# Jackxiini/Pytorch-distributed-learning

Measured on AMD Instinct MI355X. Metric: images/sec (whole node) MNIST ConvNet at 1/2/4/8 MI355X; DDP scaling efficiency, higher is better.
Workload: dtype bf16

## Files before the change

csrc/kernels/convnet.hip:

```cpp
#include <algorithm>
#include <cstdlib>
#include <type_traits>
#include <vector>

#include <cstdio>
#include <cstdlib>

#include "device_common.h"
#include "kernels.h"
#include "sgd_device.h"

namespace ringdp {
namespace kern {

using namespace ringdp::dev;

namespace {

__host__ __device__ constexpr int cdiv(int a, int b) { return (a + b - 1) / b; }

constexpr int P1_OFF = 0, P1_N = 2 * 2 * 512;
constexpr int P2F_OFF = P1_OFF + P1_N, P2F_N = 4 * 9 * 512;
constexpr int P3F_OFF = P2F_OFF + P2F_N, P3F_N = 8 * 18 * 512;
constexpr int P2D_OFF = P3F_OFF + P3F_N, P2D_N = 2 * 18 * 512;
// ... 2046 lines not shown
  __shared__ __attribute__((aligned(16))) uint8_t lds[C1W_LDS];
  bf16* xs = reinterpret_cast<bf16*>(lds + C1W_XS);
  const int tid = threadIdx.x, lane = tid & 63, wave = tid >> 6;
  const int i16 = lane & 15, g = lane >> 4, q = i16 >> 2, p = i16 & 3;
  const int t1 = 16 + i16;
  const int xoff0 = (i16 % 5) * C1W_CS + (i16 / 5) * C1W_RS + 8 * g;
  const int xoff1 = t1 < 25 ? (t1 % 5) * C1W_CS + (t1 / 5) * C1W_RS + 8 * g : 0;
  const uint32_t b1fill = t1 == 25 ? 0x3f803f80u : 0u;
  for (int i = tid; i < C1W_C / 16; i += 256) reinterpret_cast<uint4*>(lds)[i] = make_uint4(0, 0, 0, 0);
  const int per = cdiv(B, nslices);
  const int b_lo = min(B, blockIdx.x * per), b_hi = min(B, b_lo + per);
  auto dma = [&](int bb, int k) {
    const bf16* src = da1 + (int64_t)bb * C1A_IMG;
    uint8_t* dd = lds + C1W_D + k * C1W_DSZ;
    for (int i = wave; i < 11; i += 4) {
      const int c = i * 64 + lane;
      if (c < C1A_IMG / 8) glds16_async(src + c * 8, dd + i * 1024);
    }
    const uint8_t* cs = idx1 + (int64_t)bb * C1I_IMG;
    uint8_t* cd = lds + C1W_C + k * C1I_IMG;
    for (int i = wave; i < 7; i += 4) {
      const int c = i * 64 + lane;
      if (c < C1I_IMG / 16) glds16_async(cs + c * 16, cd + i * 1024);
    }
  };
  f32x4 acc[2][2];
#pragma unroll
  for (int m = 0; m < 2; ++m) acc[m][0] = acc[m][1] = zero_f32x4();
  uint32_t xu = 0;
  float4 xf = make_float4(0.f, 0.f, 0.f, 0.f);
  __syncthreads();
  if (b_lo < b_hi) {
    c1_load<U8>(xin, b_lo, tid, xu, xf);
    dma(b_lo, 0);
    c1_store<U8, 5, C1W_RS, C1W_CS>(xs, tid, xu, xf, mean, inv_std, in_scale);
  }
  int cur = 0;
  for (int b = b_lo; b < b_hi; ++b) {
    c_dma_wait();
    __syncthreads();
    if (b + 1 < b_hi) {
      c1_load<U8>(xin, b + 1, tid, xu, xf);
      dma(b + 1, cur ^ 1);
    }
    const bf16* D = reinterpret_cast<const bf16*>(lds + C1W_D + cur * C1W_DSZ);
    const uint8_t* CB = lds + C1W_C + cur * C1I_IMG;
    const int dy = wave & 1;
    for (int ks = wave; ks < 26; ks += 4) {
      const int py = ks >> 1;
      bf16x8 A[2];
#pragma unroll
      for (int m = 0; m < 2; ++m) {
        const uint2 d = __builtin_bit_cast(uint2, lds_read_tr16(D + (py * 13 + 4 * g + q) * 32 + m * 16 + 4 * p));
        const int co = m * 16 + i16;
        const uint32_t cu = *reinterpret_cast<const uint32_t*>(CB + py * 256 + (co >> 1) * 16 + 4 * g);
        const int csh = 4 * (co & 1) + 2 * dy;
        uint32_t pr[4];
#pragma unroll
        for (int k = 0; k < 4; ++k) {
          const uint32_t dv = k & 1 ? (k < 2 ? d.x : d.y) >> 16 : (k < 2 ? d.x : d.y) & 0xffffu;
          const uint32_t sel = __builtin_amdgcn_ubfe(cu, 8 * k + csh, 2);
          pr[k] = dv * ((sel * 0x8001u) & 0x10001u);
        }
        A[m] = __builtin_bit_cast(bf16x8, make_uint4(pr[0], pr[1], pr[2], pr[3]));
      }
      const bf16x8 B0 = *reinterpret_cast<const bf16x8*>(xs + xoff0 + ks * C1W_RS);
      bf16x8 B1 = *reinterpret_cast<const bf16x8*>(xs + xoff1 + ks * C1W_RS);
      if (t1 >= 25) B1 = __builtin_bit_cast(bf16x8, make_uint4(b1fill, b1fill, b1fill, b1fill));
#pragma unroll
      for (int m = 0; m < 2; ++m) {
        acc[m][0] = mfma16x16x32(A[m], B0, acc[m][0]);
        acc[m][1] = mfma16x16x32(A[m], B1, acc[m][1]);
      }
    }
    if (b + 1 < b_hi) {
      __syncthreads();
      c1_store<U8, 5, C1W_RS, C1W_CS>(xs, tid, xu, xf, mean, inv_std, in_scale);
    }
    cur ^= 1;
  }
  __syncthreads();
  float* red = reinterpret_cast<float*>(lds);
#pragma unroll
  for (int m = 0; m < 2; ++m)
#pragma unroll
    for (int n = 0; n < 2; ++n)
      *reinterpret_cast<f32x4*>(red + ((wave * 4 + m * 2 + n) * 64 + lane) * 4) = acc[m][n];
  __syncthreads();
  const int tile = tid >> 6;
  f32x4 sum = *reinterpret_cast<const f32x4*>(red + (tile * 64 + lane) * 4);
#pragma unroll
  for (int w = 1; w < 4; ++w) sum += *reinterpret_cast<const f32x4*>(red + ((w * 4 + tile) * 64 + lane) * 4);
  float* slab = slabs + (int64_t)blockIdx.x * C1_WSLAB;
  const int tap = (tile & 1) * 16 + i16;
#pragma unroll
  for (int r = 0; r < 4; ++r) {
    const int co = (tile >> 1) * 16 + g * 4 + r;
    if (tap < 25) slab[co * 25 + tap] = sum[r];
    if (tap == 25) slab[800 + co] = sum[r];
  }
}

constexpr int C12_O = 172 * C2_ORS * 2;
constexpr int C12_XS = 5 * C1W_CS * 2;
constexpr int C12_OFF_O = C2D_P, C12_OFF_X = C12_OFF_O + 2 * C12_O, C12_OFF_C = C12_OFF_X + 2 * C12_XS;
constexpr int C12_LDS = C12_OFF_C + 2 * C1I_IMG;
constexpr int C12B_LDS = C12_LDS > (C2W_D + C2W_X) ? C12_LDS : (C2W_D + C2W_X);
static_assert(C2D_P % 16 == 0 && C12_O % 16 == 0 && C12_XS % 16 == 0, "16-B aligned LDS buffers");
static_assert(8 * 4 * 64 * 4 * 4 <= C12_OFF_X, "conv1 cross-wave reduction fits in P + O");

template <bool U8>
__device__ __forceinline__ void conv12_dgrad_role(char* smem, const void* __restrict__ xin, const uint8_t* __restrict__ idx1,
                                  const bf16* __restrict__ dz2, const bf16* __restrict__ packed, int B, int block,
                                  int nblocks, float mean, float inv_std, float in_scale,
                                  float* __restrict__ slabs1) {
  bf16* P = reinterpret_cast<bf16*>(smem);
  auto Obuf = [&](int k) { return reinterpret_cast<bf16*>(smem + C12_OFF_O + k * C12_O); };
  auto Xbuf = [&](int k) { return reinterpret_cast<bf16*>(smem + C12_OFF_X + k * C12_XS); };
  auto Cbuf = [&](int k) { return reinterpret_cast<uint8_t*>(smem + C12_OFF_C + k * C1I_IMG); };
  const int tid = threadIdx.x, lane = tid & 63, wave = tid >> 6;
  const int nt = wave & 1, mg = wave >> 1;
  const int r16 = lane & 15, q8 = (lane >> 4) * 8;
  const bf16x8* pk = reinterpret_cast<const bf16x8*>(packed + P2D_OFF);
  bf16x8 bw[18];
#pragma unroll
  for (int ks = 0; ks < 18; ++ks) bw[ks] = pk[(nt * 18 + ks) * 64 + lane];
  int base[3];
  int opos[3][4];
#pragma unroll
  for (int k = 0; k < 3; ++k) {
    const int mt = min(mg + 4 * k, 10);
    const int mm = c2d_tile_pos[mt * 16 + r16] == 255 ? 0 : c2d_tile_pos[mt * 16 + r16];
    base[k] = (mm / 13) * C2_PW + mm % 13;
#pragma unroll
    for (int i = 0; i < 4; ++i) opos[k][i] = c2d_tile_pos[mt * 16 + (lane >> 4) * 4 + i];
  }
  const int i16 = lane & 15, g = lane >> 4, q = i16 >> 2, p = i16 & 3;
  const int t1 = 16 + i16;
  const int xoff0 = (i16 % 5) * C1W_CS + (i16 / 5) * C1W_RS + 8 * g;
  const int xoff1 = t1 < 25 ? (t1 % 5) * C1W_CS + (t1 / 5) * C1W_RS + 8 * g : 0;
  const uint32_t b1fill = t1 == 25 ? 0x3f803f80u : 0u;
  const int dy = wave & 1;
  f32x4 acc1[2][2];
#pragma unroll
  for (int m = 0; m < 2; ++m) acc1[m][0] = acc1[m][1] = zero_f32x4();
  for (int c = tid; c < C12_OFF_C / 16; c += 512) reinterpret_cast<bf16x8*>(smem)[c] = zero_bf16x8();
  bf16x8 pz[2];
  uint4 pc = make_uint4(0, 0, 0, 0);
  uint32_t xu = 0;
  float4 xf = make_float4(0.f, 0.f, 0.f, 0.f);
  auto load = [&](int bb) {
    const bf16x8* src = reinterpret_cast<const bf16x8*>(dz2 + (int64_t)bb * 121 * 64);
    pz[0] = src[tid];
    if (tid + 512 < 968) pz[1] = src[tid + 512];
    if (tid < C1I_IMG / 16) pc = reinterpret_cast<const uint4*>(idx1 + (int64_t)bb * C1I_IMG)[tid];
    c1_load<U8>(xin, bb, tid, xu, xf);
  };
  auto stage = [&](int k) {
#pragma unroll
    for (int j = 0; j < 2; ++j) {
      const int c = tid + 512 * j;
      if (c < 968) {
        const int pos = c >> 3, cc = (c & 7) * 8;
        *reinterpret_cast<bf16x8*>(P + ((pos / 11 + 2) * C2_PW + pos % 11 + 2) * C2_PRS + cc) = pz[j];
      }
    }
    if (tid < C1I_IMG / 16) reinterpret_cast<uint4*>(Cbuf(k))[tid] = pc;
    c1_store<U8, 5, C1W_RS, C1W_CS>(Xbuf(k), tid, xu, xf, mean, inv_std, in_scale);
  };
  auto c1_step = [&](int j, int k) {
    const int ks0 = wave + 8 * j;
    const bool ok = ks0 < 26;
    const int ks = ok ? ks0 : 0;
    const int py = ks >> 1;
    const bf16* O = Obuf(k);
    const bf16* xs = Xbuf(k);
    const uint8_t* CB = Cbuf(k);
    bf16x8 A[2];
#pragma unroll
    for (int m = 0; m < 2; ++m) {
      const uint2 d = __builtin_bit_cast(uint2, lds_read_tr16(O + (py * 13 + 4 * g + q) * C2_ORS + m * 16 + 4 * p));
      const int co = m * 16 + i16;
      const uint32_t cu = *reinterpret_cast<const uint32_t*>(CB + py * 256 + (co >> 1) * 16 + 4 * g);
      const int csh = 4 * (co & 1) + 2 * dy;
      uint32_t pr[4];
#pragma unroll
      for (int e = 0; e < 4; ++e) {
        const uint32_t dv = e & 1 ? (e < 2 ? d.x : d.y) >> 16 : (e < 2 ? d.x : d.y) & 0xffffu;
        const uint32_t sel = __builtin_amdgcn_ubfe(cu, 8 * e + csh, 2);
        pr[e] = ok ? dv * ((sel * 0x8001u) & 0x10001u) : 0u;
      }
      A[m] = __builtin_bit_cast(bf16x8, make_uint4(pr[0], pr[1], pr[2], pr[3]));
    }
    const bf16x8 B0 = *reinterpret_cast<const bf16x8*>(xs + xoff0 + ks * C1W_RS);
    bf16x8 B1 = *reinterpret_cast<const bf16x8*>(xs + xoff1 + ks * C1W_RS);
    if (t1 >= 25) B1 = __builtin_bit_cast(bf16x8, make_uint4(b1fill, b1fill, b1fill, b1fill));
#pragma unroll
    for (int m = 0; m < 2; ++m) {
      acc1[m][0] = mfma16x16x32(A[m], B0, acc1[m][0]);
      acc1[m][1] = mfma16x16x32(A[m], B1, acc1[m][1]);
    }
  };
  auto phase = [&](auto nk_c, auto c1_c, int k) {
    constexpr int NK = decltype(nk_c)::value;
    constexpr bool C1 = decltype(c1_c)::value;
    f32x4 acc[NK];
#pragma unroll
    for (int m = 0; m < NK; ++m) acc[m] = zero_f32x4();
#pragma unroll
    for (int ks = 0; ks < 18; ++ks) {
      const int tapp = ks >> 1, c0 = (ks & 1) * 32;
      const int shift = (tapp / 3) * C2_PW + tapp % 3;
#pragma unroll
      for (int m = 0; m < NK; ++m)
        acc[m] = mfma16x16x32(*reinterpret_cast<const bf16x8*>(P + (base[m] + shift) * C2_PRS + c0 + q8), bw[ks],
                              acc[m]);
      if (C1 && (ks & 3) == 3 && ks < 16) c1_step(ks >> 2, k ^ 1);
    }
    bf16* O = Obuf(k);
#pragma unroll
    for (int m = 0; m < NK; ++m) {
#pragma unroll
      for (int i = 0; i < 4; ++i) {
        const int pos = opos[m][i];
        if (pos < 169) O[pos * C2_ORS + nt * 16 + r16] = (bf16)acc[m][i];
      }
    }
  };
  using I2 = std::integral_constant<int, 2>;
  using I3 = std::integral_constant<int, 3>;
  using T = std::true_type;
  using Fa = std::false_type;
  __syncthreads();
  int b = block, k = 0;
  if (b < B) load(b);
  for (int i = 0; b < B; ++i, b += nblocks, k ^= 1) {
    __syncthreads();
    stage(k);
    const int nb = b + nblocks;
    if (nb < B) load(nb);
    __syncthreads();
    if (i == 0) {
      if (mg < 3) phase(I3{}, Fa{}, k);
      else phase(I2{}, Fa{}, k);
    } else {
      if (mg < 3) phase(I3{}, T{}, k);
      else phase(I2{}, T{}, k);
    }
  }
  __syncthreads();
  if (b != block) {
#pragma unroll
    for (int j = 0; j < 4; ++j) c1_step(j, k ^ 1);
  }
  __syncthreads();
  float* red = reinterpret_cast<float*>(smem);
#pragma unroll
  for (int m = 0; m < 2; ++m)
#pragma unroll
    for (int n = 0; n < 2; ++n)
      *reinterpret_cast<f32x4*>(red + ((wave * 4 + m * 2 + n) * 64 + lane) * 4) = acc1[m][n];
  __syncthreads();
  if (tid >= 256) return;
  const int tile = tid >> 6;
  f32x4 sum = *reinterpret_cast<const f32x4*>(red + (tile * 64 + lane) * 4);
#pragma unroll
  for (int w = 1; w < 8; ++w) sum += *reinterpret_cast<const f32x4*>(red + ((w * 4 + tile) * 64 + lane) * 4);
  float* slab = slabs1 + (int64_t)block * C1_WSLAB;
  const int tap = (tile & 1) * 16 + i16;
#pragma unroll
  for (int r = 0; r < 4; ++r) {
    const int co = (tile >> 1) * 16 + g * 4 + r;
    if (tap < 25) slab[co * 25 + tap] = sum[r];
    if (tap == 25) slab[800 + co] = sum[r];
  }
}

template <bool U8>
__global__ __launch_bounds__(512) void conv12_bwd_kernel(const void* __restrict__ xin,
                                                         const uint8_t* __restrict__ idx1,
                                                         const bf16* __restrict__ a1,
                                                         const bf16* __restrict__ dz2,
                                                         const bf16* __restrict__ packed, int B,
                                                         float mean, float inv_std, float in_scale,
                                                         float* __restrict__ slabs2, int nslices,
                                                         float* __restrict__ slabs1, int n_dgrad) {
  __shared__ __attribute__((aligned(16))) char smem[C12B_LDS];
  if ((int)blockIdx.x < n_dgrad)
    conv12_dgrad_role<U8>(smem, xin, idx1, dz2, packed, B, blockIdx.x, n_dgrad, mean, inv_std, in_scale, slabs1);
  else
    conv2_wgrad_role(smem, a1, dz2, slabs2, B, nslices, blockIdx.x - n_dgrad);
}

constexpr int C12V_DG = 2 * (C2D_P + C12_O) + 3 * (C12_XS + C1I_IMG);
constexpr int C12V_WG = 3 * (C2W_D + C2W_X);
constexpr int C12V_LDS = C12V_DG > C12V_WG ? C12V_DG : C12V_WG;
static_assert(C12V_LDS <= 160 * 1024 && C1I_IMG % 16 == 0, "conv12 backward (8-wave) LDS");

#ifndef RINGDP_C12_ABLATE
#define RINGDP_C12_ABLATE 0
#endif
constexpr int C12_ABLATE = RINGDP_C12_ABLATE;

template <bool U8>
__device__ __forceinline__ void conv12_dgrad8_role(char* smem, const void* __restrict__ xin,
                                                   const uint8_t* __restrict__ idx1, const bf16* __restrict__ dz2,
                                                   const bf16* __restrict__ packed, int B, int block, int nblocks,
                                                   float mean, float inv_std, float in_scale,
                                                   float* __restrict__ slabs1, int ablate) {
  auto Pb = [&](int k) { return reinterpret_cast<bf16*>(smem + k * C2D_P); };
  auto Ob = [&](int k) { return reinterpret_cast<bf16*>(smem + 2 * C2D_P + k * C12_O); };
  auto Xb = [&](int k) { return reinterpret_cast<bf16*>(smem + 2 * (C2D_P + C12_O) + k * C12_XS); };
  auto Cb = [&](int k) { return reinterpret_cast<uint8_t*>(smem + 2 * (C2D_P + C12_O) + 3 * C12_XS + k * C1I_IMG); };
  const int tid = threadIdx.x, lane = tid & 63;
  const int wave = __builtin_amdgcn_readfirstlane(tid >> 6);
  const int n = block < B ? (B - block + nblocks - 1) / nblocks : 0;
  for (int c = tid; c < (2 * (C2D_P + C12_O) + 3 * C12_XS) / 16; c += 512)
    reinterpret_cast<bf16x8*>(smem)[c] = zero_bf16x8();
  __syncthreads();
  if ((ablate & 8) && wave >= 4) __builtin_amdgcn_s_setprio(1);
  if (wave < 4) {
    const int r16 = lane & 15, q8 = (lane >> 4) * 8, c4 = (lane >> 4) * 4;
    const bf16x8* pk = reinterpret_cast<const bf16x8*>(packed + P2D_OFF);
    bf16x8 bw[2][18];
#pragma unroll
    for (int nt = 0; nt < 2; ++nt)
#pragma unroll
      for (int ks = 0; ks < 18; ++ks) bw[nt][ks] = pk[(nt * 18 + ks) * 64 + lane];
    int base[3], opos[3];
#pragma unroll
    for (int k = 0; k < 3; ++k) {
      const int mt = min(wave + 4 * k, 10);
      const int mm = c2d_tile_pos[mt * 16 + r16];
      opos[k] = mm;
      base[k] = mm == 255 ? 0 : (mm / 13) * C2_PW + mm % 13;
    }
    auto phase = [&](auto nk_c, const bf16* P, bf16* O) {
      constexpr int NK = decltype(nk_c)::value;
      f32x4 acc[NK][2];
#pragma unroll
      for (int k = 0; k < NK; ++k) acc[k][0] = acc[k][1] = zero_f32x4();
#pragma unroll
      for (int ks = 0; ks < 18; ++ks) {
        const int tapp = ks >> 1, c0 = (ks & 1) * 32;
        const int shift = (tapp / 3) * C2_PW + tapp % 3;
#pragma unroll
        for (int k = 0; k < NK; ++k) {
          const bf16x8 a = *reinterpret_cast<const bf16x8*>(P + (base[k] + shift) * C2_PRS + c0 + q8);
          acc[k][0] = mfma16x16x32(bw[0][ks], a, acc[k][0]);
          acc[k][1] = mfma16x16x32(bw[1][ks], a, acc[k][1]);
        }
      }
#pragma unroll
      for (int k = 0; k < NK; ++k) {
        if (opos[k] < 169) {
#pragma unroll
          for (int nt = 0; nt < 2; ++nt)
            *reinterpret_cast<bf16x4*>(O + opos[k] * C2_ORS + nt * 16 + c4) =
                bf16x4{(bf16)acc[k][nt][0], (bf16)acc[k][nt][1], (bf16)acc[k][nt][2], (bf16)acc[k][nt][3]};
        }
      }
    };
    lds_barrier();
    for (int s = 0; s <= n; ++s) {
      if (s < n && !(ablate & 2)) {
        if (wave < 3)
          phase(std::integral_constant<int, 3>{}, Pb(s & 1), Ob(s & 1));
        else
          phase(std::integral_constant<int, 2>{}, Pb(s & 1), Ob(s & 1));
      }
      lds_barrier();
    }
    __syncthreads();
    __syncthreads();
  } else {
    const int vt = tid - 256, vw = wave - 4;
    const int i16 = lane & 15, g = lane >> 4, q = i16 >> 2, p = i16 & 3;
    const int t1 = 16 + i16;
    const int xoff0 = (i16 % 5) * C1W_CS + (i16 / 5) * C1W_RS + 8 * g;
    const int xoff1 = t1 < 25 ? (t1 % 5) * C1W_CS + (t1 / 5) * C1W_RS + 8 * g : 0;
    const uint32_t b1fill = t1 == 25 ? 0x3f803f80u : 0u;
    const int dy = vw & 1;
    f32x4 acc1[2][2];
#pragma unroll
    for (int m = 0; m < 2; ++m) acc1[m][0] = acc1[m][1] = zero_f32x4();
    struct Regs {
      bf16x8 pz[4];
      uint4 pc;
      uint32_t xu;
      float4 xf;
    };
    Regs r0, r1;
    auto load = [&](Regs& r, int bb) {
      const bf16x8* src = reinterpret_cast<const bf16x8*>(dz2 + (int64_t)bb * 121 * 64);
#pragma unroll
      for (int j = 0; j < 4; ++j)
        if (vt + 256 * j < 968) r.pz[j] = src[vt + 256 * j];
      if (vt < C1I_IMG / 16) r.pc = reinterpret_cast<const uint4*>(idx1 + (int64_t)bb * C1I_IMG)[vt];
      c1_load<U8>(xin, bb, vt, r.xu, r.xf);
    };
    auto stage = [&](const Regs& r, int k2, int k3) {
      bf16* P = Pb(k2);
#pragma unroll
      for (int j = 0; j < 4; ++j) {
        const int c = vt + 256 * j;
        if (c < 968) {
          const int pos = c >> 3, cc = (c & 7) * 8;
          *reinterpret_cast<bf16x8*>(P + ((pos / 11 + 2) * C2_PW + pos % 11 + 2) * C2_PRS + cc) = r.pz[j];
        }
      }
      if (vt < C1I_IMG / 16) reinterpret_cast<uint4*>(Cb(k3))[vt] = r.pc;
      c1_store<U8, 5, C1W_RS, C1W_CS>(Xb(k3), vt, r.xu, r.xf, mean, inv_std, in_scale);
    };
    auto c1_step = [&](int ks, const bf16* O, const bf16* xs, const uint8_t* CB) {
      const int py = ks >> 1;
      bf16x8 A[2];
#pragma unroll
      for (int m = 0; m < 2; ++m) {
        const uint2 d = __builtin_bit_cast(uint2, lds_read_tr16(O + (py * 13 + 4 * g + q) * C2_ORS + m * 16 + 4 * p));
        const int co = m * 16 + i16;
        const uint32_t cu = *reinterpret_cast<const uint32_t*>(CB + py * 256 + (co >> 1) * 16 + 4 * g);
        const int csh = 4 * (co & 1) + 2 * dy;
        uint32_t pr[4];
#pragma unroll
        for (int e = 0; e < 4; ++e) {
          const uint32_t dv = e & 1 ? (e < 2 ? d.x : d.y) >> 16 : (e < 2 ? d.x : d.y) & 0xffffu;
          const uint32_t sel = __builtin_amdgcn_ubfe(cu, 8 * e + csh, 2);
          pr[e] = dv * ((sel * 0x8001u) & 0x10001u);
        }
        A[m] = __builtin_bit_cast(bf16x8, make_uint4(pr[0], pr[1], pr[2], pr[3]));
      }
      const bf16x8 B0 = *reinterpret_cast<const bf16x8*>(xs + xoff0 + ks * C1W_RS);
      bf16x8 B1 = *reinterpret_cast<const bf16x8*>(xs + xoff1 + ks * C1W_RS);
      if (t1 >= 25) B1 = __builtin_bit_cast(bf16x8, make_uint4(b1fill, b1fill, b1fill, b1fill));
#pragma unroll
      for (int m = 0; m < 2; ++m) {
        acc1[m][0] = mfma16x16x32(A[m], B0, acc1[m][0]);
        acc1[m][1] = mfma16x16x32(A[m], B1, acc1[m][1]);
      }
    };
    if (n > 0) {
      load(r0, block);
      stage(r0, 0, 0);
      if (n > 1) load(r1, block + nblocks);
      if (n > 2) load(r0, block + 2 * nblocks);
    }
    lds_barrier();
    auto step = [&](int s, Regs& rs) {
      if (s + 1 < n) {
        stage(rs, (s + 1) & 1, (s + 1) % 3);
        if (s + 3 < n) load(rs, block + (s + 3) * nblocks);
      }
      if (s >= 1 && !(ablate & 1)) {
        const bf16* O = Ob((s - 1) & 1);
        const bf16* xs = Xb((s - 1) % 3);
        const uint8_t* CB = Cb((s - 1) % 3);
        for (int ks = vw; ks < 26; ks += 4) c1_step(ks, O, xs, CB);
      }
      lds_barrier();
    };
    for (int s = 0; s <= n; s += 2) {
      step(s, r1);
      if (s + 1 <= n) step(s + 1, r0);
    }
    __syncthreads();
    float* red = reinterpret_cast<float*>(smem);
#pragma unroll
    for (int m = 0; m < 2; ++m)
#pragma unroll
      for (int nn = 0; nn < 2; ++nn)
        *reinterpret_cast<f32x4*>(red + ((vw * 4 + m * 2 + nn) * 64 + lane) * 4) = acc1[m][nn];
    __syncthreads();
    const int tile = vw;
    f32x4 sum = *reinterpret_cast<const f32x4*>(red + (tile * 64 + lane) * 4);
#pragma unroll
    for (int w = 1; w < 4; ++w) sum += *reinterpret_cast<const f32x4*>(red + ((w * 4 + tile) * 64 + lane) * 4);
    float* slab = slabs1 + (int64_t)block * C1_WSLAB;
    const int tap = (tile & 1) * 16 + i16;
#pragma unroll
    for (int r = 0; r < 4; ++r) {
      const int co = (tile >> 1) * 16 + g * 4 + r;
      if (tap < 25) slab[co * 25 + tap] = sum[r];
      if (tap == 25) slab[800 + co] = sum[r];
    }
  }
}

__device__ __forceinline__ void conv2_wgrad8_role(char* smem, const bf16* __restrict__ a1, const bf16* __restrict__ dz2,
                                                  float* __restrict__ slabs, int B, int nslices, int slice) {
  auto Db = [&](int k) { return reinterpret_cast<bf16*>(smem + k * C2W_D); };
  auto Xb = [&](int k) { return reinterpret_cast<bf16*>(smem + 3 * C2W_D + k * C2W_X); };
  const int tid = threadIdx.x, lane = tid & 63;
  const int wave = __builtin_amdgcn_readfirstlane(tid >> 6);
  const int wm2 = wave & 1, wn = wave >> 1, half = wn & 1, h = wn >> 1;
  const int g16 = lane & 15, grp = lane >> 4, q = g16 >> 2, p = g16 & 3;
  const bf16x8 onesf = ones_column_frag(lane);
  f32x4 acc[2][5], accb[2];
#pragma unroll
  for (int m = 0; m < 2; ++m) {
    accb[m] = zero_f32x4();
#pragma unroll
    for (int j = 0; j < 5; ++j) acc[m][j] = zero_f32x4();
  }
  for (int c = tid; c < 3 * C2W_D / 16; c += 512) reinterpret_cast<bf16x8*>(smem)[c] = zero_bf16x8();
  const int n = slice < B ? (B - slice + nslices - 1) / nslices : 0;
  auto img = [&](int i) { return slice + i * nslices; };
  struct Regs {
    bf16x8 pz[2], pa[2];
  };
  Regs r0, r1;
  auto load = [&](Regs& r, int bb) {
    const bf16x8* zs = reinterpret_cast<const bf16x8*>(dz2 + (int64_t)bb * 121 * 64);
    const bf16x8* as = reinterpret_cast<const bf16x8*>(a1 + (int64_t)bb * 169 * 32);
    r.pz[0] = zs[tid];
    if (tid + 512 < 968) r.pz[1] = zs[tid + 512];
    r.pa[0] = as[tid];
    if (tid + 512 < 676) r.pa[1] = as[tid + 512];
  };
  auto stage = [&](const Regs& r, int k) {
    bf16* D = Db(k);
    bf16* X = Xb(k);
#pragma unroll
    for (int j = 0; j < 2; ++j) {
      const int c = tid + 512 * j;
      if (c < 968) *reinterpret_cast<bf16x8*>(D + c2_drow(c >> 3) + (c & 7) * 8) = r.pz[j];
      if (c < 676) *reinterpret_cast<bf16x8*>(X + (c >> 2) * C2_XRS + (c & 3) * 8) = r.pa[j];
    }
  };
  auto readA = [&](int buf, int ks, bf16x8 (&af)[2]) {
    const bf16* D = Db(buf) + 32 * wm2 + 4 * p;
    const int kb = ks * 32 + grp * 8;
#pragma unroll
    for (int m = 0; m < 2; ++m) {
      const bf16x4 alo = lds_read_tr16(D + c2_drow(kb + q) + m * 16);
      const bf16x4 ahi = lds_read_tr16(D + c2_drow(kb + 4 + q) + m * 16);
      af[m] = bf16x8{alo[0], alo[1], alo[2], alo[3], ahi[0], ahi[1], ahi[2], ahi[3]};
    }
  };
  __syncthreads();
  if (n > 0) {
    load(r0, img(0));
    stage(r0, 0);
    if (n > 1) {
      load(r1, img(1));
      stage(r1, 1);
    }
    if (n > 2) load(r0, img(2));
    if (n > 3) load(r1, img(3));
  }
  lds_barrier();
  bf16x8 af[2], afn[2];
  if (n > 0) readA(0, 0, af);
  auto body = [&](auto h_c) {
    constexpr int H = decltype(h_c)::value;
    constexpr int NJ = H == 0 ? 5 : 4;
    auto image = [&](int i, Regs& rs) {
      const int cur = i % 3;
      if (i + 2 < n) {
        stage(rs, (i + 2) % 3);
        if (i + 4 < n) load(rs, img(i + 4));
      }
      const int xb = (int)(Xb(cur) - reinterpret_cast<const bf16*>(smem)) + 16 * half + 4 * p;
#pragma unroll
      for (int ks = 0; ks < 4; ++ks) {
        const int kb = ks * 32 + grp * 8;
        const int k0 = min(kb + q, 120), k1 = min(kb + 4 + q, 120);
        int x0 = xb + ((k0 / 11) * 13 + k0 % 11) * C2_XRS, x1 = xb + ((k1 / 11) * 13 + k1 % 11) * C2_XRS;
        asm("" : "+v"(x0), "+v"(x1));
        const bf16* S0 = reinterpret_cast<const bf16*>(smem);
#pragma unroll
        for (int j = 0; j < NJ; ++j) {
          const int tap = 2 * j + H;
          const int shift = ((tap / 3) * 13 + tap % 3) * C2_XRS;
          const bf16x4 lo = lds_read_tr16(S0 + x0 + shift);
          const bf16x4 hi = lds_read_tr16(S0 + x1 + shift);
          const bf16x8 bf = bf16x8{lo[0], lo[1], lo[2], lo[3], hi[0], hi[1], hi[2], hi[3]};
          if (j == 2) {
            if (ks < 3) {
              if (ks & 1)
                readA(cur, ks + 1, af);
              else
                readA(cur, ks + 1, afn);
            } else if (i + 1 < n) {
              readA((i + 1) % 3, 0, af);
            }
          }
#pragma unroll
          for (int m = 0; m < 2; ++m) acc[m][j] = mfma16x16x32((ks & 1) ? afn[m] : af[m], bf, acc[m][j]);
        }
        if (wn == 0) {
#pragma unroll
          for (int m = 0; m < 2; ++m) accb[m] = mfma16x16x32((ks & 1) ? afn[m] : af[m], onesf, accb[m]);
        }
      }
      lds_barrier();
    };
    for (int i = 0; i < n; i += 2) {
      image(i, r0);
      if (i + 1 < n) image(i + 1, r1);
    }
  };
  if (h == 0)
    body(std::integral_constant<int, 0>{});
  else
    body(std::integral_constant<int, 1>{});
  float* slab = slabs + (int64_t)slice * C2_WSLAB;
  const int nj = h == 0 ? 5 : 4;
#pragma unroll
  for (int m = 0; m < 2; ++m) {
    const int co = (2 * wm2 + m) * 16 + grp * 4;
#pragma unroll
    for (int j = 0; j < 5; ++j) {
      if (j < nj) {
        const int nn = ((2 * j + h) * 2 + half) * 16 + g16;
        *reinterpret_cast<f32x4*>(slab + (int64_t)nn * 64 + co) = acc[m][j];
      }
    }
    if (wn == 0 && g16 == 0) *reinterpret_cast<f32x4*>(slab + 288 * 64 + co) = accb[m];
  }
}

template <bool U8>
__global__ __launch_bounds__(512, 1) void conv12_bwd8_kernel(const void* __restrict__ xin,
                                                            const uint8_t* __restrict__ idx1,
                                                            const bf16* __restrict__ a1,
                                                            const bf16* __restrict__ dz2,
                                                            const bf16* __restrict__ packed, int B, float mean,
                                                            float inv_std, float in_scale,
                                                            float* __restrict__ slabs2, int nslices,
                                                            float* __restrict__ slabs1, int n_dgrad, int ablate) {
  __shared__ __attribute__((aligned(16))) char smem[C12V_LDS];
  if ((int)blockIdx.x < n_dgrad)
    conv12_dgrad8_role<U8>(smem, xin, idx1, dz2, packed, B, blockIdx.x, n_dgrad, mean, inv_std, in_scale, slabs1,
                           ablate);
  else if (!(ablate & 4))
    conv2_wgrad8_role(smem, a1, dz2, slabs2, B, nslices, blockIdx.x - n_dgrad);
}

constexpr int kMaxRedSegs = 8;
struct ReduceSegs {
  ReduceSeg seg[kMaxRedSegs];
  int count;
};

constexpr int kRedWaves = 8;
__device__ __forceinline__ void red_store(const ReduceSeg& sg, int64_t i, float v) {
  if (sg.mode == 0) {
    sg.out[i] = v;
  } else if (sg.mode == 2) {
    const int t = (int)(i & 255), nj = (int)(i >> 8), n = nj >> 3, j = nj & 7;
    sg.out[n * 2048 + ((t & 15) * 8 + j) * 16 + (t >> 4)] = v;
  } else {
    const int n = (int)(i / sg.cout), co = (int)(i % sg.cout);
    sg.out[((int64_t)co * sg.cin + n % sg.cin) * 9 + n / sg.cin] = v;
  }
}

__global__ __launch_bounds__(64 * kRedWaves) void slab_reduce_kernel(ReduceSegs segs) {
  __shared__ f32x4 part[kRedWaves][64];
  int blk = blockIdx.x, sidx = 0;
  while (sidx < segs.count - 1 && blk >= segs.seg[sidx].blocks) {
    blk -= segs.seg[sidx].blocks;
    ++sidx;
  }
  const ReduceSeg& sg = segs.seg[sidx];
  const int lane = threadIdx.x & 63, wave = threadIdx.x >> 6;
  const int V = sg.vec;
  const int64_t i0 = ((int64_t)blk * 64 + lane) * V;
  f32x4 a0 = zero_f32x4(), a1 = zero_f32x4(), a2 = zero_f32x4(), a3 = zero_f32x4();
  if (i0 < sg.n) {
    const float* pp = sg.slabs + sg.off + i0;
    int s = wave;
    if (V == 4) {
      for (; s + 3 * kRedWaves < sg.nslices; s += 4 * kRedWaves) {
        a0 += *reinterpret_cast<const f32x4*>(pp + (int64_t)s * sg.stride);
        a1 += *reinterpret_cast<const f32x4*>(pp + (int64_t)(s + kRedWaves) * sg.stride);
        a2 += *reinterpret_cast<const f32x4*>(pp + (int64_t)(s + 2 * kRedWaves) * sg.stride);
        a3 += *reinterpret_cast<const f32x4*>(pp + (int64_t)(s + 3 * kRedWaves) * sg.stride);
      }
      for (; s < sg.nslices; s += kRedWaves) a0 += *reinterpret_cast<const f32x4*>(pp + (int64_t)s * sg.stride);
    } else {
      for (; s + 3 * kRedWaves < sg.nslices; s += 4 * kRedWaves) {
        a0[0] += pp[(int64_t)s * sg.stride];
        a1[0] += pp[(int64_t)(s + kRedWaves) * sg.stride];
        a2[0] += pp[(int64_t)(s + 2 * kRedWaves) * sg.stride];
        a3[0] += pp[(int64_t)(s + 3 * kRedWaves) * sg.stride];
      }
      for (; s < sg.nslices; s += kRedWaves) a0[0] += pp[(int64_t)s * sg.stride];
    }
  }
  part[wave][lane] = (a0 + a1) + (a2 + a3);
  __syncthreads();
  if (wave != 0 || i0 >= sg.n) return;
  f32x4 v = zero_f32x4();
#pragma unroll
  for (int w = 0; w < kRedWaves; ++w) v += part[w][lane];
  for (int k = 0; k < V; ++k) red_store(sg, i0 + k, v[k]);
}

ReduceSeg seg(const float* slabs, int64_t stride, int64_t off, int64_t n, int nslices, float* out,
              int mode = 0, int cin = 0, int cout = 0) {
  const int vec = ((off | stride | n) & 3) == 0 ? 4 : 1;
  return ReduceSeg{slabs, stride, off, n, nslices, out, mode, cin, cout, (int)((n + 64 * vec - 1) / (64 * vec)), vec};
}

void launch_reduce(const std::vector<ReduceSeg>& v, hipStream_t s) {
  if (v.empty()) return;
  if (v.size() > (size_t)kMaxRedSegs) {
    launch_reduce(std::vector<ReduceSeg>(v.begin(), v.begin() + kMaxRedSegs), s);
    launch_reduce(std::vector<ReduceSeg>(v.begin() + kMaxRedSegs, v.end()), s);
    return;
  }
  ReduceSegs segs{};
  int total = 0;
  segs.count = (int)v.size();
  for (size_t k = 0; k < v.size(); ++k) {
    segs.seg[k] = v[k];
    total += v[k].blocks;
  }
  slab_reduce_kernel<<<total, 64 * kRedWaves, 0, s>>>(segs);
}

int num_cus() {
  static int cus = [] {
    int dev = 0, n = 256;
    if (hipGetDevice(&dev) == hipSuccess) {
      hipDeviceProp_t p;
      if (hipGetDeviceProperties(&p, dev) == hipSuccess) n = p.multiProcessorCount;
    }
    return n;
  }();
  return cus;
}

inline int clampi(int v, int lo, int hi) { return v < lo ? lo : (v > hi ? hi : v); }

int fc_in_c3_max_batch() {
  static const int v = [] {
    const char* e = std::getenv("RINGDP_CN_FC_IN_C3_MAX");
    return e ? std::atoi(e) : 2048;
  }();
  return v;
}

int fc_fused_max_batch() {
  static const int v = [] {
    const char* e = std::getenv("RINGDP_CN_FC_FUSED_MAX");
    return e ? std::atoi(e) : 4096;
  }();
  return v;
}

int wpc(const char* name, int dflt) {
  char key[64];
  std::snprintf(key, sizeof(key), "RINGDP_CN_WPC_%s", name);
  const char* v = std::getenv(key);
  return v ? std::max(1, std::atoi(v)) : dflt;
}

}

int64_t cn_packed_elems() { return PACK_TOTAL; }

void cn_pack_weights(const float* w1, const float* w2, const float* w3, const float* wfc, void* out,
                     hipStream_t s) {
  pack_weights_kernel<<<cdiv(PACK_TOTAL, 1024), 256, 0, s>>>(PackSrc{w1, w2, w3, wfc}, static_cast<bf16*>(out));
}

void cn_conv1_fwd(const void* x, bool u8, const void* packed, const float* b1, void* a1, uint8_t* idx1,
                  int B, float mean, float inv_std, float in_scale, hipStream_t s, const float* const* pack_w,
                  void* pack_out) {
  const int grid = clampi(B, 1, wpc("C1F", 3) * num_cus());
  const bf16* pk = static_cast<const bf16*>(packed);
  bf16* a1b = static_cast<bf16*>(a1);
  if (pack_w) {
    const PackSrc ws{pack_w[0], pack_w[1], pack_w[2], pack_w[3]};
    const int g = grid + cdiv(PACK_TOTAL, 1024);
    bf16* po = static_cast<bf16*>(pack_out);
    if (u8)
      conv1_fwd_kernel<true, true><<<g, 256, 0, s>>>(x, pk, b1, a1b, idx1, B, mean, inv_std, in_scale, ws, po, grid);
    else
      conv1_fwd_kernel<false, true><<<g, 256, 0, s>>>(x, pk, b1, a1b, idx1, B, mean, inv_std, in_scale, ws, po, grid);
    return;
  }
  const PackSrc none{nullptr, nullptr, nullptr, nullptr};
  if (u8)
    conv1_fwd_kernel<true, false><<<grid, 256, 0, s>>>(x, pk, b1, a1b, idx1, B, mean, inv_std, in_scale, none, nullptr, grid);
  else
    conv1_fwd_kernel<false, false><<<grid, 256, 0, s>>>(x, pk, b1, a1b, idx1, B, mean, inv_std, in_scale, none, nullptr, grid);
}

void cn_sgd_flat_pack(float* p, const float* g, float* m, int64_t n, const SgdArgs& a, const int64_t* offsets,
                      void* packed, hipStream_t s) {
  if (n <= 0) return;
  PackDst d{static_cast<bf16*>(packed), {offsets[0], offsets[1], offsets[2], offsets[3]}};
  const int grid = std::max<int64_t>(1, std::min<int64_t>((n / 4 + 256) / 256, 2048));
  if (m && a.momentum != 0.f)
    cn_sgd_pack_kernel<true><<<grid, 256, 0, s>>>(p, g, m, n, a, d);
  else
    cn_sgd_pack_kernel<false><<<grid, 256, 0, s>>>(p, g, m, n, a, d);
}

void cn_forward_fused(const void* x, bool u8, const float* const* w, const float* b1, const float* b2,
                      const float* b3, const float* bfc, void* packed, void* a1, uint8_t* idx1, void* a2,
                      uint8_t* idx2, void* a3, uint8_t* idx3, float* logits, int B, float mean, float inv_std,
                      float in_scale, hipStream_t s, bool do_pack) {
  const int grid = clampi(B, 1, wpc("FF", 1) * num_cus());
  bf16* pk = static_cast<bf16*>(packed);
  bf16 *a1b = static_cast<bf16*>(a1), *a2b = static_cast<bf16*>(a2), *a3b = static_cast<bf16*>(a3);
  if (do_pack) pack_weights_kernel<<<cdiv(PACK_TOTAL, 1024), 256, 0, s>>>(PackSrc{w[0], w[1], w[2], w[3]}, pk);
  const bool fc_in = B <= fc_fused_max_batch();
  float* lg = fc_in ? logits : nullptr;
  if (u8)
    fused_fwd_kernel<true><<<grid, 512, 0, s>>>(x, pk, b1, b2, b3, bfc, a1b, idx1, a2b, idx2, a3b, idx3, lg, B, mean,
                                                inv_std, in_scale);
  else
    fused_fwd_kernel<false><<<grid, 512, 0, s>>>(x, pk, b1, b2, b3, bfc, a1b, idx1, a2b, idx2, a3b, idx3, lg, B, mean,
                                                 inv_std, in_scale);
  if (!fc_in) fc1_fwd_kernel<<<cdiv(B, 16 * FC1_G), 256, 0, s>>>(a3b, pk, bfc, logits, B);
}

void cn_conv2_fwd(const void* a1, const void* packed, const float* b2, void* a2, uint8_t* idx2, int B,
                  hipStream_t s) {
  const int grid = clampi(B, 1, wpc("C2F", 3) * num_cus());
  conv2_fwd_kernel<<<grid, 256, 0, s>>>(static_cast<const bf16*>(a1), static_cast<const bf16*>(packed), b2,
                                        static_cast<bf16*>(a2), idx2, B);
}

void cn_conv3_fc_fwd(const void* a2, const void* packed, const float* b3, const float* bfc, float* logits,
                     void* a3, uint8_t* idx3, int B, hipStream_t s) {
  const int grid = clampi(B, 1, wpc("C3F", 2) * num_cus());
  const bf16* a2b = static_cast<const bf16*>(a2);
  const bf16* pk = static_cast<const bf16*>(packed);
  if (B <= fc_fused_max_batch()) {
    conv3_fwd_kernel<true><<<grid, 256, 0, s>>>(a2b, pk, b3, static_cast<bf16*>(a3), idx3, B, bfc, logits);
    return;
  }
  conv3_fwd_kernel<false><<<grid, 256, 0, s>>>(a2b, pk, b3, static_cast<bf16*>(a3), idx3, B, nullptr, nullptr);
  fc1_fwd_kernel<<<cdiv(B, 16 * FC1_G), 256, 0, s>>>(static_cast<const bf16*>(a3), pk, bfc, logits, B);
}

static double split_frac(const char* env, double dflt) {
  const char* v = getenv(env);
  if (!v) return dflt;
  const double f = atof(v);
  return f > 0.05 && f < 0.95 ? f : dflt;
}

static int min_slab_images(const char* env, int dflt) {
  const char* v = getenv(env);
  const int n = v ? atoi(v) : dflt;
  return n >= 1 && n <= 64 ? n : dflt;
}

static bool c3_v3(int B) { return B > fc_in_c3_max_batch(); }

static void c3_split(int B, bool dgrad, int& nd, int& ws) {
  if (c3_v3(B)) {
    const int cus = num_cus();
    static const double frac = split_frac("RINGDP_C3_DGRAD_FRAC", 0.55);
    nd = clampi(((int)(frac * cus) + 4) / 8 * 8, 8, cus - 8);
    ws = clampi(cdiv(B, 8), 1, cus - nd);
    if (!dgrad) nd = 0;
    return;
  }
  const int slots = 2 * num_cus();
  if (!dgrad) {
    nd = 0;
    ws = clampi(cdiv(B, 8), 1, slots / 2);
    return;
  }
  static const double frac = split_frac("RINGDP_C3_DGRAD_FRAC", 0.5);
  static const int wmin = min_slab_images("RINGDP_C3_WMIN", 2);
  nd = clampi(B, 1, (int)(frac * slots));
  const int per = cdiv(B, nd);
  ws = clampi(cdiv(B, std::max(per, wmin)), 1, std::max(1, (slots - nd) / 2));
}

static int c3_dgrad_images(int B, int nd) {
  static const double steal = [] {
    const char* v = getenv("RINGDP_C3_STEAL");
    const double f = v ? atof(v) : 0.04;
    return f >= 0.0 && f < 0.9 ? f : 0.04;
  }();
  if (nd <= 0 || B < 32 * nd) return B;
  return B - (int)(steal * B);
}

static void c2_split(int B, bool dgrad, int& nd, int& ws) {
  const int cus = num_cus();
  if (!dgrad) {
    nd = 0;
    ws = clampi(cdiv(B, 8), 1, cus);
    return;
  }
  static const double frac = split_frac("RINGDP_C2_DGRAD_FRAC", 0.55);
  nd = clampi(B, 1, (int)(frac * cus));
  const int per = cdiv(B, nd);
  ws = clampi(cdiv(B, std::max(per, 2)), 1, std::max(1, cus - nd));
}

static bool c12_v3(int B) { return B > fc_in_c3_max_batch(); }

static void c12_split(int B, int& nd, int& ws) {
  const int cus = num_cus();
  if (c12_v3(B)) {
    static const double frac3 = split_frac("RINGDP_C12_DGRAD_FRAC", 0.65);
    nd = clampi(((int)(frac3 * cus) + 4) / 8 * 8, 8, cus - 8);
    ws = clampi(cdiv(B, 8), 1, cus - nd);
    return;
  }
  static const double frac = split_frac("RINGDP_C12_DGRAD_FRAC", 0.64);
  static const int wmin = min_slab_images("RINGDP_C12_WMIN", 2);
  nd = clampi(B, 1, (int)(frac * cus));
  const int per = cdiv(B, nd);
  ws = clampi(cdiv(B, std::max(per, wmin)), 1, std::max(1, cus - nd));
}

static int conv1_wslices(int B) { return clampi(cdiv(B, 4), 1, 3 * num_cus()); }

static int fc_imgs_host(int B) {
  static const int forced = [] {
    const char* v = getenv("RINGDP_CN_FC_IMGS");
    return v && *v ? atoi(v) : 0;
  }();
  return forced > 0 ? std::min(forced, 128) : fc_imgs(B);
}
int64_t cn_fc_slab_floats(int B, bool) { return (int64_t)cdiv(B, fc_imgs_host(B)) * FC_SLAB; }
int64_t cn_conv3_slab_floats(int B, bool dgrad) {
  int nd, ws;
  c3_split(B, dgrad, nd, ws);
  return (int64_t)ws * C3_WSLAB;
}
int64_t cn_conv2_slab_floats(int B, bool dgrad) {
  int nd, ws;
  c2_split(B, dgrad, nd, ws);
  return (int64_t)ws * C2_WSLAB;
}
int64_t cn_conv12_slab_floats(int B) {
  int nd, ws;
  c12_split(B, nd, ws);
  return (int64_t)ws * C2_WSLAB + (int64_t)nd * C1_WSLAB;
}
int64_t cn_conv1_slab_floats(int B) { return (int64_t)conv1_wslices(B) * C1_WSLAB; }

void cn_conv3_fc_bwd(const void* a2, const uint8_t* idx2, const void* a3, const uint8_t* idx3, const float* wfc,
                     const float* dl, const void* packed, void* da3m, void* dz2, int B, float* fc_slabs,
                     float* c3_slabs, float* dw3, float* db3, float* dwfc, float* dbfc, hipStream_t s,
                     const CeFuse* ce, ReduceList* defer) {
  (void)wfc;
  int nd, ws;
  c3_split(B, dz2 != nullptr, nd, ws);
  const int fs = cdiv(B, fc_imgs_host(B));
  const bf16* a3b = static_cast<const bf16*>(a3);
  const bf16* pk = static_cast<const bf16*>(packed);
  const CeFuse cef = ce ? *ce : CeFuse{};
  if (!c3_v3(B)) {
    const C3Src src{a3b, pk, ce ? nullptr : dl, cef};
    conv3_bwd_kernel<<<fs + nd + 2 * ws, 256, 0, s>>>(static_cast<const bf16*>(a2), idx2, src, idx3, pk,
                                                       static_cast<bf16*>(dz2), B, c3_slabs, ws, nd,
                                                       c3_dgrad_images(B, nd), fs, fc_slabs, fc_imgs_host(B));
  } else {
    if (ce)
      fc_bwd_kernel<true><<<fs, 256, 0, s>>>(a3b, pk, nullptr, static_cast<bf16*>(da3m), fc_slabs, B, fc_imgs_host(B), cef);
    else
      fc_bwd_kernel<false><<<fs, 256, 0, s>>>(a3b, pk, dl, static_cast<bf16*>(da3m), fc_slabs, B, fc_imgs_host(B), cef);
    conv3_bwd8_kernel<<<nd + ws, 512, 0, s>>>(static_cast<const bf16*>(a2), idx2, static_cast<const bf16*>(da3m), idx3,
                                             pk, static_cast<bf16*>(dz2), B, c3_slabs, ws, nd, c3_dgrad_images(B, nd));
  }
  ReduceList r{seg(c3_slabs, C3_WSLAB, 0, 576 * 128, ws, dw3, 1, 64, 128),
               seg(fc_slabs, FC_SLAB, 20490, 128, fs, db3), seg(fc_slabs, FC_SLAB, 0, 20480, fs, dwfc, 2),
               seg(fc_slabs, FC_SLAB, 20480, 10, fs, dbfc)};
  if (defer)
    defer->insert(defer->end(), r.begin(), r.end());
  else
    launch_reduce(r, s);
}

void cn_launch_reduce(const ReduceList& segs, hipStream_t s) { launch_reduce(segs, s); }

void cn_conv2_bwd(const void* a1, const void* dz2, const void* packed, void* da1, int B, float* slabs,
                  float* dw2, float* db2, hipStream_t s) {
  int nd, ws;
  c2_split(B, da1 != nullptr, nd, ws);
  conv2_bwd_kernel<<<nd + ws, 512, 0, s>>>(static_cast<const bf16*>(a1), static_cast<const bf16*>(dz2),
                                           static_cast<const bf16*>(packed), static_cast<bf16*>(da1), B, slabs,
                                           ws, nd);
  launch_reduce({seg(slabs, C2_WSLAB, 0, 288 * 64, ws, dw2, 1, 32, 64), seg(slabs, C2_WSLAB, 288 * 64, 64, ws, db2)},
                s);
}

void cn_conv12_bwd(const void* x, bool u8, const uint8_t* idx1, const void* a1, const void* dz2,
                   const void* packed, int B, float mean, float inv_std, float in_scale, float* slabs, float* dw2,
                   float* db2, float* dw1, float* db1, hipStream_t s, const ReduceList* extra) {
  int nd, ws;
  c12_split(B, nd, ws);
  float* slabs2 = slabs;
  float* slabs1 = slabs + (int64_t)ws * C2_WSLAB;
  const bf16* a1b = static_cast<const bf16*>(a1);
  const bf16* dzb = static_cast<const bf16*>(dz2);
  const bf16* pk = static_cast<const bf16*>(packed);
  if (c12_v3(B)) {
    if (u8)
      conv12_bwd8_kernel<true><<<nd + ws, 512, 0, s>>>(x, idx1, a1b, dzb, pk, B, mean, inv_std, in_scale, slabs2, ws,
                                                       slabs1, nd, C12_ABLATE);
    else
      conv12_bwd8_kernel<false><<<nd + ws, 512, 0, s>>>(x, idx1, a1b, dzb, pk, B, mean, inv_std, in_scale, slabs2, ws,
                                                        slabs1, nd, C12_ABLATE);
  } else if (u8)
    conv12_bwd_kernel<true><<<nd + ws, 512, 0, s>>>(x, idx1, a1b, dzb, pk, B, mean, inv_std, in_scale, slabs2, ws,
                                                    slabs1, nd);
  else
    conv12_bwd_kernel<false><<<nd + ws, 512, 0, s>>>(x, idx1, a1b, dzb, pk, B, mean, inv_std, in_scale, slabs2, ws,
                                                     slabs1, nd);
  ReduceList r = extra ? *extra : ReduceList{};
  for (const ReduceSeg& g : {seg(slabs2, C2_WSLAB, 0, 288 * 64, ws, dw2, 1, 32, 64),
                             seg(slabs2, C2_WSLAB, 288 * 64, 64, ws, db2), seg(slabs1, C1_WSLAB, 0, 800, nd, dw1),
                             seg(slabs1, C1_WSLAB, 800, 32, nd, db1)})
    r.push_back(g);
  launch_reduce(r, s);
}

void cn_conv1_wgrad(const void* x, bool u8, const void* da1, const uint8_t* idx1, int B, float mean,
                    float inv_std, float in_scale, float* slabs, float* dw1, float* db1, hipStream_t s) {
  const int ws = conv1_wslices(B);
  if (u8)
    conv1_wgrad_kernel<true><<<ws, 256, 0, s>>>(x, static_cast<const bf16*>(da1), idx1, B, mean, inv_std, in_scale,
                                                slabs, ws);
  else
    conv1_wgrad_kernel<false><<<ws, 256, 0, s>>>(x, static_cast<const bf16*>(da1), idx1, B, mean, inv_std, in_scale,
                                                 slabs, ws);
  launch_reduce({seg(slabs, C1_WSLAB, 0, 800, ws, dw1), seg(slabs, C1_WSLAB, 800, 32, ws, db1)}, s);
}

}
}
```

Baseline: 20.38 million.

## Spread conv1 wgrad k-steps across all eight waves in conv12 dgrad role

The conv1 weight-gradient MFMA work, which used to run only on the four staging waves, is now partitioned over all eight waves. The conv2-dgrad waves take a few k-steps each after their phase, and the cross-wave reduction is widened to sum eight partials. In the wgrad role, the late waves now do their staging after the MFMA loop so the staging work is staggered. The dgrad CU fraction default is lowered to rebalance against wgrad, and optional timestamp instrumentation is added behind a macro.

```diff
diff --git a/csrc/kernels/convnet.hip b/csrc/kernels/convnet.hip
--- a/csrc/kernels/convnet.hip
+++ b/csrc/kernels/convnet.hip
@@ -2372,6 +2372,21 @@
 #endif
 constexpr int C12_ABLATE = RINGDP_C12_ABLATE;
 
+#ifdef RINGDP_C12_STAMPS
+constexpr int C12_ST_S0 = 100, C12_ST_BLK = 5, C12_ST_BYTES = 8 * 8 * 4 * 8;
+#define C12_ST(s, k)                                                                                              \
+  do {                                                                                                            \
+    if ((s) >= C12_ST_S0 && (s) < C12_ST_S0 + 8 && (threadIdx.x & 63) == 0)                                       \
+      reinterpret_cast<unsigned long long*>(smem + C12V_LDS)[((threadIdx.x >> 6) * 8 + ((s) - C12_ST_S0)) * 4 + (k)] = \
+          __builtin_amdgcn_s_memtime();                                                                           \
+  } while (0)
+#else
+constexpr int C12_ST_BYTES = 0;
+#define C12_ST(s, k) \
+  do {               \
+  } while (0)
+#endif
+
 template <bool U8>
 __device__ __forceinline__ void conv12_dgrad8_role(char* smem, const void* __restrict__ xin,
                                                    const uint8_t* __restrict__ idx1, const bf16* __restrict__ dz2,
@@ -2389,6 +2404,72 @@
     reinterpret_cast<bf16x8*>(smem)[c] = zero_bf16x8();
   __syncthreads();
   if ((ablate & 8) && wave >= 4) __builtin_amdgcn_s_setprio(1);
+  constexpr int C12_KM = 2, C12_KM3 = 4, C12_KH = 26 - 3 * C12_KM - C12_KM3;
+  static_assert(C12_KH >= 4 && C12_KM >= 0 && C12_KM3 >= 0, "conv1 k-step partition");
+  const int k0 = wave < 4 ? C12_KH + wave * C12_KM : wave - 4, kst = wave < 4 ? 1 : 4;
+  const int kcnt = wave < 3 ? C12_KM : wave == 3 ? C12_KM3 : (C12_KH - (wave - 4) + 3) / 4;
+  const int i16 = lane & 15, g = lane >> 4, q = i16 >> 2, p = i16 & 3;
+  const int t1 = 16 + i16;
+  const int xoff0 = (i16 % 5) * C1W_CS + (i16 / 5) * C1W_RS + 8 * g;
+  const int xoff1 = t1 < 25 ? (t1 % 5) * C1W_CS + (t1 / 5) * C1W_RS + 8 * g : 0;
+  const uint32_t b1fill = t1 == 25 ? 0x3f803f80u : 0u;
+  f32x4 acc1[2][2];
+#pragma unroll
+  for (int m = 0; m < 2; ++m) acc1[m][0] = acc1[m][1] = zero_f32x4();
+  const int o_lane = ((4 * g + q) * C2_ORS + 4 * p) * 2;
+  const int c_lane = (i16 >> 1) * 16 + 4 * g, csh_lane = 4 * (i16 & 1);
+  struct C1F {
+    uint2 d[2];
+    uint32_t cu[2];
+    bf16x8 b0, b1;
+  };
+  auto c1_read = [&](int ks, int oimg, int ximg, int cimg, C1F& f) {
+    const int py = ks >> 1;
+    int oa = oimg + py * (13 * C2_ORS * 2) + o_lane, ca = cimg + py * 256 + c_lane;
+    int x0 = ximg + ks * (C1W_RS * 2) + xoff0 * 2, x1 = ximg + ks * (C1W_RS * 2) + xoff1 * 2;
+    asm("" : "+v"(oa), "+v"(ca), "+v"(x0), "+v"(x1));
+#pragma unroll
+    for (int m = 0; m < 2; ++m) {
+      f.d[m] = __builtin_bit_cast(uint2, lds_read_tr16(reinterpret_cast<const bf16*>(smem + oa) + m * 16));
+      f.cu[m] = *reinterpret_cast<const uint32_t*>(smem + ca + m * 128);
+    }
+    f.b0 = *reinterpret_cast<const bf16x8*>(smem + x0);
+    f.b1 = *reinterpret_cast<const bf16x8*>(smem + x1);
+  };
+  auto c1_mma = [&](int ks, const C1F& f) {
+    bf16x8 A[2];
+    const int csh = csh_lane + 2 * (ks & 1);
+#pragma unroll
+    for (int m = 0; m < 2; ++m) {
+      const uint2 d = f.d[m];
+      const uint32_t cu = f.cu[m];
+      uint32_t pr[4];
+#pragma unroll
+      for (int e = 0; e < 4; ++e) {
+        const uint32_t dv = e & 1 ? (e < 2 ? d.x : d.y) >> 16 : (e < 2 ? d.x : d.y) & 0xffffu;
+        const uint32_t sel = __builtin_amdgcn_ubfe(cu, 8 * e + csh, 2);
+        pr[e] = dv * ((sel * 0x8001u) & 0x10001u);
+      }
+      A[m] = __builtin_bit_cast(bf16x8, make_uint4(pr[0], pr[1], pr[2], pr[3]));
+    }
+    bf16x8 B1 = f.b1;
+    if (t1 >= 25) B1 = __builtin_bit_cast(bf16x8, make_uint4(b1fill, b1fill, b1fill, b1fill));
+#pragma unroll
+    for (int m = 0; m < 2; ++m) {
+      acc1[m][0] = mfma16x16x32(A[m], f.b0, acc1[m][0]);
+      acc1[m][1] = mfma16x16x32(A[m], B1, acc1[m][1]);
+    }
+  };
+  auto c1_image = [&](int j) {
+    const int oimg = 2 * C2D_P + (j & 1) * C12_O;
+    const int ximg = 2 * (C2D_P + C12_O) + (j % 3) * C12_XS;
+    const int cimg = 2 * (C2D_P + C12_O) + 3 * C12_XS + (j % 3) * C1I_IMG;
+    for (int i = 0, ks = k0; i < kcnt; ++i, ks += kst) {
+      C1F f;
+      c1_read(ks, oimg, ximg, cimg, f);
+      c1_mma(ks, f);
+    }
+  };
   if (wave < 4) {
     const int r16 = lane & 15, q8 = (lane >> 4) * 8, c4 = (lane >> 4) * 4;
     const bf16x8* pk = reinterpret_cast<const bf16x8*>(packed + P2D_OFF);
@@ -2405,7 +2486,7 @@
       opos[k] = mm;
       base[k] = mm == 255 ? 0 : (mm / 13) * C2_PW + mm % 13;
     }
-    auto phase = [&](auto nk_c, const bf16* P, bf16* O) {
+    auto phase = [&](auto nk_c, const bf16* P, bf16* O, int s) {
       constexpr int NK = decltype(nk_c)::value;
       f32x4 acc[NK][2];
 #pragma unroll
@@ -2421,6 +2502,7 @@
           acc[k][1] = mfma16x16x32(bw[1][ks], a, acc[k][1]);
         }
       }
+      C12_ST(s, 1);
 #pragma unroll
       for (int k = 0; k < NK; ++k) {
         if (opos[k] < 169) {
@@ -2433,27 +2515,20 @@
     };
     lds_barrier();
     for (int s = 0; s <= n; ++s) {
+      C12_ST(s, 0);
       if (s < n && !(ablate & 2)) {
         if (wave < 3)
-          phase(std::integral_constant<int, 3>{}, Pb(s & 1), Ob(s & 1));
+          phase(std::integral_constant<int, 3>{}, Pb(s & 1), Ob(s & 1), s);
         else
-          phase(std::integral_constant<int, 2>{}, Pb(s & 1), Ob(s & 1));
-      }
+          phase(std::integral_constant<int, 2>{}, Pb(s & 1), Ob(s & 1), s);
+      }
+      C12_ST(s, 2);
+      if (s >= 1 && !(ablate & 1)) c1_image(s - 1);
+      C12_ST(s, 3);
       lds_barrier();
     }
-    __syncthreads();
-    __syncthreads();
   } else {
-    const int vt = tid - 256, vw = wave - 4;
-    const int i16 = lane & 15, g = lane >> 4, q = i16 >> 2, p = i16 & 3;
-    const int t1 = 16 + i16;
-    const int xoff0 = (i16 % 5) * C1W_CS + (i16 / 5) * C1W_RS + 8 * g;
-    const int xoff1 = t1 < 25 ? (t1 % 5) * C1W_CS + (t1 / 5) * C1W_RS + 8 * g : 0;
-    const uint32_t b1fill = t1 == 25 ? 0x3f803f80u : 0u;
-    const int dy = vw & 1;
-    f32x4 acc1[2][2];
-#pragma unroll
-    for (int m = 0; m < 2; ++m) acc1[m][0] = acc1[m][1] = zero_f32x4();
+    const int vt = tid - 256;
     struct Regs {
       bf16x8 pz[4];
       uint4 pc;
@@ -2482,33 +2557,6 @@
       if (vt < C1I_IMG / 16) reinterpret_cast<uint4*>(Cb(k3))[vt] = r.pc;
       c1_store<U8, 5, C1W_RS, C1W_CS>(Xb(k3), vt, r.xu, r.xf, mean, inv_std, in_scale);
     };
-    auto c1_step = [&](int ks, const bf16* O, const bf16* xs, const uint8_t* CB) {
-      const int py = ks >> 1;
-      bf16x8 A[2];
-#pragma unroll
-      for (int m = 0; m < 2; ++m) {
-        const uint2 d = __builtin_bit_cast(uint2, lds_read_tr16(O + (py * 13 + 4 * g + q) * C2_ORS + m * 16 + 4 * p));
-        const int co = m * 16 + i16;
-        const uint32_t cu = *reinterpret_cast<const uint32_t*>(CB + py * 256 + (co >> 1) * 16 + 4 * g);
-        const int csh = 4 * (co & 1) + 2 * dy;
-        uint32_t pr[4];
-#pragma unroll
-        for (int e = 0; e < 4; ++e) {
-          const uint32_t dv = e & 1 ? (e < 2 ? d.x : d.y) >> 16 : (e < 2 ? d.x : d.y) & 0xffffu;
-          const uint32_t sel = __builtin_amdgcn_ubfe(cu, 8 * e + csh, 2);
-          pr[e] = dv * ((sel * 0x8001u) & 0x10001u);
-        }
-        A[m] = __builtin_bit_cast(bf16x8, make_uint4(pr[0], pr[1], pr[2], pr[3]));
-      }
-      const bf16x8 B0 = *reinterpret_cast<const bf16x8*>(xs + xoff0 + ks * C1W_RS);
-      bf16x8 B1 = *reinterpret_cast<const bf16x8*>(xs + xoff1 + ks * C1W_RS);
-      if (t1 >= 25) B1 = __builtin_bit_cast(bf16x8, make_uint4(b1fill, b1fill, b1fill, b1fill));
-#pragma unroll
-      for (int m = 0; m < 2; ++m) {
-        acc1[m][0] = mfma16x16x32(A[m], B0, acc1[m][0]);
-        acc1[m][1] = mfma16x16x32(A[m], B1, acc1[m][1]);
-      }
-    };
     if (n > 0) {
       load(r0, block);
       stage(r0, 0, 0);
@@ -2519,32 +2567,33 @@
     auto step = [&](int s, Regs& rs) {
       if (s + 1 < n) {
         stage(rs, (s + 1) & 1, (s + 1) % 3);
+        C12_ST(s, 0);
         if (s + 3 < n) load(rs, block + (s + 3) * nblocks);
       }
-      if (s >= 1 && !(ablate & 1)) {
-        const bf16* O = Ob((s - 1) & 1);
-        const bf16* xs = Xb((s - 1) % 3);
-        const uint8_t* CB = Cb((s - 1) % 3);
-        for (int ks = vw; ks < 26; ks += 4) c1_step(ks, O, xs, CB);
-      }
+      C12_ST(s, 1);
+      if (s >= 1 && !(ablate & 1)) c1_image(s - 1);
+      C12_ST(s, 2);
       lds_barrier();
+      C12_ST(s, 3);
     };
     for (int s = 0; s <= n; s += 2) {
       step(s, r1);
       if (s + 1 <= n) step(s + 1, r0);
     }
-    __syncthreads();
-    float* red = reinterpret_cast<float*>(smem);
-#pragma unroll
-    for (int m = 0; m < 2; ++m)
-#pragma unroll
-      for (int nn = 0; nn < 2; ++nn)
-        *reinterpret_cast<f32x4*>(red + ((vw * 4 + m * 2 + nn) * 64 + lane) * 4) = acc1[m][nn];
-    __syncthreads();
-    const int tile = vw;
+  }
+  __syncthreads();
+  float* red = reinterpret_cast<float*>(smem);
+#pragma unroll
+  for (int m = 0; m < 2; ++m)
+#pragma unroll
+    for (int nn = 0; nn < 2; ++nn)
+      *reinterpret_cast<f32x4*>(red + ((wave * 4 + m * 2 + nn) * 64 + lane) * 4) = acc1[m][nn];
+  __syncthreads();
+  if (wave >= 4) {
+    const int tile = wave - 4;
     f32x4 sum = *reinterpret_cast<const f32x4*>(red + (tile * 64 + lane) * 4);
 #pragma unroll
-    for (int w = 1; w < 4; ++w) sum += *reinterpret_cast<const f32x4*>(red + ((w * 4 + tile) * 64 + lane) * 4);
+    for (int w = 1; w < 8; ++w) sum += *reinterpret_cast<const f32x4*>(red + ((w * 4 + tile) * 64 + lane) * 4);
     float* slab = slabs1 + (int64_t)block * C1_WSLAB;
     const int tap = (tile & 1) * 16 + i16;
 #pragma unroll
@@ -2626,10 +2675,12 @@
     constexpr int NJ = H == 0 ? 5 : 4;
     auto image = [&](int i, Regs& rs) {
       const int cur = i % 3;
-      if (i + 2 < n) {
+      const bool early = wave < 4;
+      if (early && i + 2 < n) {
         stage(rs, (i + 2) % 3);
         if (i + 4 < n) load(rs, img(i + 4));
       }
+      C12_ST(i, 0);
       const int xb = (int)(Xb(cur) - reinterpret_cast<const bf16*>(smem)) + 16 * half + 4 * p;
 #pragma unroll
       for (int ks = 0; ks < 4; ++ks) {
@@ -2663,7 +2714,13 @@
           for (int m = 0; m < 2; ++m) accb[m] = mfma16x16x32((ks & 1) ? afn[m] : af[m], onesf, accb[m]);
         }
       }
+      C12_ST(i, 1);
+      if (!early && i + 2 < n) {
+        stage(rs, (i + 2) % 3);
+        if (i + 4 < n) load(rs, img(i + 4));
+      }
       lds_barrier();
+      C12_ST(i, 2);
     };
     for (int i = 0; i < n; i += 2) {
       image(i, r0);
@@ -2699,12 +2756,27 @@
                                                             float inv_std, float in_scale,
                                                             float* __restrict__ slabs2, int nslices,
                                                             float* __restrict__ slabs1, int n_dgrad, int ablate) {
-  __shared__ __attribute__((aligned(16))) char smem[C12V_LDS];
+  __shared__ __attribute__((aligned(16))) char smem[C12V_LDS + C12_ST_BYTES];
   if ((int)blockIdx.x < n_dgrad)
     conv12_dgrad8_role<U8>(smem, xin, idx1, dz2, packed, B, blockIdx.x, n_dgrad, mean, inv_std, in_scale, slabs1,
                            ablate);
   else if (!(ablate & 4))
     conv2_wgrad8_role(smem, a1, dz2, slabs2, B, nslices, blockIdx.x - n_dgrad);
+#ifdef RINGDP_C12_STAMPS
+  __syncthreads();
+  const bool dg = (int)blockIdx.x < n_dgrad;
+  const int blk = dg ? blockIdx.x : blockIdx.x - n_dgrad, nb = dg ? n_dgrad : nslices;
+  if (blk == C12_ST_BLK && threadIdx.x == 0 && (B - blk) / nb > C12_ST_S0 + 8) {
+    const unsigned long long* st = reinterpret_cast<const unsigned long long*>(smem + C12V_LDS);
+    const unsigned long long t0 = st[0];
+    for (int w = 0; w < 8; ++w)
+      for (int k = 0; k < 8; ++k) {
+        const unsigned long long* r = st + (w * 8 + k) * 4;
+        printf("C12ST %c w%d s%d %lld %lld %lld %lld\n", dg ? 'd' : 'w', w, k, (long long)(r[0] - t0),
+               (long long)(r[1] - t0), (long long)(r[2] - t0), dg ? (long long)(r[3] - t0) : 0ll);
+      }
+  }
+#endif
 }
 
 constexpr int kMaxRedSegs = 8;
@@ -2975,7 +3047,7 @@
 static void c12_split(int B, int& nd, int& ws) {
   const int cus = num_cus();
   if (c12_v3(B)) {
-    static const double frac3 = split_frac("RINGDP_C12_DGRAD_FRAC", 0.65);
+    static const double frac3 = split_frac("RINGDP_C12_DGRAD_FRAC", 0.59);
     nd = clampi(((int)(frac3 * cus) + 4) / 8 * 8, 8, cus - 8);
     ws = clampi(cdiv(B, 8), 1, cus - nd);
     return;
```

After: 20.60 million (median of 6 runs). 1.1% higher.
